# kelaendi/mused

Measured on AMD Instinct MI355X. Metric: stream rows/sec, d=1024 l=128 window=10k synthetic (SWFD + kNN similarity + eigenstep + labels), higher is better.
Workload: dtype f64; 1 GPU; synthetic d=1024 l=128 window=10000 k=50 (BASELINE config 2); stream=blob, W=10000, d=1024, l=128, k=50, modalities=1, swfd_levels=14, rccl_ranks=1, lanes_per_gpu=20, padded_window_slots=2

## Files before the change

mused_amd/csrc/gemm_f64.h:

```cpp
#pragma once
#include <cstdlib>
#include <mutex>
#include <type_traits>
#include "common.h"

namespace mused {

typedef double v4f64 __attribute__((ext_vector_type(4)));

constexpr int GEMM_BM = 128;
constexpr int GEMM_BN = 128;
constexpr int GEMM_BK = 16;
constexpr int GEMM_LD = 144;
constexpr int GEMM_THREADS = 256;
constexpr int GEMM_LDS_BYTES = 2  * 2  * GEMM_BK * GEMM_LD * 8;

struct GemmArgs {
  const void* A;
  const void* B;
  long lda, ldb;
  long strideA, strideB;
  int M, N, K;
  int kchunk;
  int splitk;
  int bsplit;
  int tiles_m, tiles_n;
  const int* rep;
  const int* list;
  const int* kact;
  int sym;
};

template <typename TIn, bool VEC>
__device__ __forceinline__ void stage_load_kc(const TIn* __restrict__ src, long ld, int r0, int nrows, int k0,
                                              int kend, TIn (&r)[8]) {
  const int m = threadIdx.x & 127;
  const int kh = threadIdx.x >> 7;
  const int row = r0 + m;
  const int k = k0 + kh * 8;
  if (row < nrows) {
    const TIn* p = src + (long)row * ld + k;
    if (VEC && k + 8 <= kend) {
      if (sizeof(TIn) == 4) {
        const float4 a = *reinterpret_cast<const float4*>(p);
        const float4 b = *reinterpret_cast<const float4*>(p + 4);
        r[0] = a.x; r[1] = a.y; r[2] = a.z; r[3] = a.w;
        r[4] = b.x; r[5] = b.y; r[6] = b.z; r[7] = b.w;
      } else {
        const double2* q = reinterpret_cast<const double2*>(p);
#pragma unroll
        for (int j = 0; j < 4; ++j) {
          const double2 v = q[j];
          r[2 * j] = v.x;
          r[2 * j + 1] = v.y;
        }
      }
    } else {
#pragma unroll
      for (int j = 0; j < 8; ++j) r[j] = (k + j < kend) ? p[j] : (TIn)0;
    }
  } else {
#pragma unroll
    for (int j = 0; j < 8; ++j) r[j] = (TIn)0;
// ... 52 lines not shown

template <typename TIn>
__device__ __forceinline__ void stage_load8(const TIn* __restrict__ p, TIn (&r)[8]) {
  if (sizeof(TIn) == 4) {
    const float4 a = *reinterpret_cast<const float4*>(p);
    const float4 b = *reinterpret_cast<const float4*>(p + 4);
    r[0] = a.x; r[1] = a.y; r[2] = a.z; r[3] = a.w;
    r[4] = b.x; r[5] = b.y; r[6] = b.z; r[7] = b.w;
  } else {
    const double2* q = reinterpret_cast<const double2*>(p);
#pragma unroll
    for (int j = 0; j < 4; ++j) {
      const double2 v = q[j];
      r[2 * j] = v.x;
      r[2 * j + 1] = v.y;
    }
  }
}
template <typename TIn>
__device__ __forceinline__ void stage_load_kc_full(const TIn* __restrict__ src, long ld, int r0, int k0, TIn (&r)[8]) {
  stage_load8(src + (long)(r0 + (threadIdx.x & 127)) * ld + k0 + (threadIdx.x >> 7) * 8, r);
}
template <typename TIn>
__device__ __forceinline__ void stage_load_mc_full(const TIn* __restrict__ src, long ld, int c0, int k0, TIn (&r)[8]) {
  stage_load8(src + (long)(k0 + (threadIdx.x >> 4)) * ld + c0 + (threadIdx.x & 15) * 8, r);
}

__device__ __forceinline__ int xcd_remap(int pid, int nwg) {
  const int q = nwg >> 3, r = nwg & 7, xcd = pid & 7;
  const int base = (xcd < r) ? xcd * (q + 1) : r * (q + 1) + (xcd - r) * q;
  return base + (pid >> 3);
}

template <typename TA, typename TB, bool A_KC, bool B_KC, bool VEC>
__device__ __forceinline__ void gemm_tile_mainloop(const GemmArgs& g, const TA* __restrict__ A, const TB* __restrict__ B,
                                                   int m0, int n0, int k_lo, int k_hi, double* smem,
                                                   v4f64 (&acc)[4][4]) {
  double* As = smem;
  double* Bs = smem + 2 * GEMM_BK * GEMM_LD;
  const int lane = threadIdx.x & 63;
  const int wave = threadIdx.x >> 6;
  const int wr = wave >> 1, wc = wave & 1;
  const int kq = lane >> 4, li = lane & 15;
#pragma unroll
  for (int i = 0; i < 4; ++i)
#pragma unroll
    for (int j = 0; j < 4; ++j) acc[i][j] = (v4f64){0.0, 0.0, 0.0, 0.0};

  TA ra[8];
  TB rb[8];
  const int nkt = (k_hi - k_lo + GEMM_BK - 1) / GEMM_BK;

  const bool full_mn = VEC && m0 + GEMM_BM <= g.M && n0 + GEMM_BN <= g.N;
  auto load_tile = [&](int kt) {
    const int k0 = k_lo + kt * GEMM_BK;
    if (full_mn && k0 + GEMM_BK <= k_hi) {
      if (A_KC) stage_load_kc_full<TA>(A, g.lda, m0, k0, ra); else stage_load_mc_full<TA>(A, g.lda, m0, k0, ra);
      if (B_KC) stage_load_kc_full<TB>(B, g.ldb, n0, k0, rb); else stage_load_mc_full<TB>(B, g.ldb, n0, k0, rb);
      return;
    }
    if (A_KC) stage_load_kc<TA, VEC>(A, g.lda, m0, g.M, k0, k_hi, ra);
    else      stage_load_mc<TA, VEC>(A, g.lda, m0, g.M, k0, k_hi, ra);
    if (B_KC) stage_load_kc<TB, VEC>(B, g.ldb, n0, g.N, k0, k_hi, rb);
    else      stage_load_mc<TB, VEC>(B, g.ldb, n0, g.N, k0, k_hi, rb);
  };
  auto store_tile = [&](int buf) {
    double* a = As + buf * GEMM_BK * GEMM_LD;
    double* b = Bs + buf * GEMM_BK * GEMM_LD;
    if (A_KC) stage_store_kc(a, ra); else stage_store_mc(a, ra);
    if (B_KC) stage_store_kc(b, rb); else stage_store_mc(b, rb);
  };

  if (nkt > 0) {
    load_tile(0);
    store_tile(0);
  }
  __syncthreads();

  int cur = 0;
  for (int kt = 0; kt < nkt; ++kt) {
    const bool more = (kt + 1 < nkt);
    if (more) load_tile(kt + 1);
    const double* a = As + cur * GEMM_BK * GEMM_LD + wr * 64 + li;
    const double* b = Bs + cur * GEMM_BK * GEMM_LD + wc * 64 + li;
#pragma unroll
    for (int kk = 0; kk < GEMM_BK / 4; ++kk) {
      double fa[4], fb[4];
#pragma unroll
      for (int i = 0; i < 4; ++i) fa[i] = a[(kk * 4 + kq) * GEMM_LD + i * 16];
#pragma unroll
      for (int j = 0; j < 4; ++j) fb[j] = b[(kk * 4 + kq) * GEMM_LD + j * 16];
#pragma unroll
      for (int i = 0; i < 4; ++i)
#pragma unroll
        for (int j = 0; j < 4; ++j)
          acc[i][j] = __builtin_amdgcn_mfma_f64_16x16x4f64(fa[i], fb[j], acc[i][j], 0, 0, 0);
    }
    if (more) store_tile(cur ^ 1);
    __syncthreads();
    cur ^= 1;
  }
}

constexpr int DIAG_I[4][9] = {{0, 0, 1, 0, 1, 2, 0, 1, 2}, {3, 0, 1, 2, 3, 4, 0, 1, 2}, {3, 4, 5, 0, 1, 2, 3, 4, 5}, {6, 0, 1, 2, 3, 4, 5, 6, 7}};
constexpr int DIAG_J[4][9] = {{0, 1, 1, 2, 2, 2, 3, 3, 3}, {3, 4, 4, 4, 4, 4, 5, 5, 5}, {5, 5, 5, 6, 6, 6, 6, 6, 6}, {6, 7, 7, 7, 7, 7, 7, 7, 7}};
constexpr int DIAG_NF[4] = {4, 6, 7, 8};
constexpr int DIAG_NGRP[4] = {3, 2, 2, 1};
constexpr int DIAG_GRP[4][3][3] = {{{1, 0, 1}, {2, 0, 2}, {3, 0, 3}}, {{4, 0, 4}, {5, 0, 3}, {0, 0, 0}}, {{5, 3, 2}, {6, 0, 6}, {0, 0, 0}}, {{7, 0, 7}, {0, 0, 0}, {0, 0, 0}}};
constexpr int DIAG_PATCH_LD = 130;

constexpr int diag_acc_index(int w, int i, int j) {
  for (int n = 0; n < 9; ++n)
    if (DIAG_I[w][n] == i && DIAG_J[w][n] == j) return n;
  return -1;
}

template <int W, int N = 0>
__device__ __forceinline__ void diag_mfma9(const double (&f)[8], v4f64 (&acc)[9]) {
  if constexpr (N < 9) {
    constexpr int i = DIAG_I[W][N], j = DIAG_J[W][N];
    acc[N] = __builtin_amdgcn_mfma_f64_16x16x4f64(f[i], f[j], acc[N], 0, 0, 0);
    diag_mfma9<W, N + 1>(f, acc);
  }
}
template <int W>
__device__ __forceinline__ void diag_kstep(const double* __restrict__ a, v4f64 (&acc)[9]) {
#pragma unroll
  for (int kk = 0; kk < GEMM_BK / 4; ++kk) {
    double f[8];
#pragma unroll
    for (int b = 0; b < 8; ++b) f[b] = (b < DIAG_NF[W]) ? a[kk * 4 * GEMM_LD + b * 16] : 0.0;
    diag_mfma9<W>(f, acc);
  }
}

template <typename TA, bool A_KC, bool VEC>
__device__ __forceinline__ void gemm_tile_mainloop_diag(const GemmArgs& g, const TA* __restrict__ A, int m0, int k_lo, int k_hi,
                                                        double* As, int wave, v4f64 (&acc)[9]) {
  const int lane = threadIdx.x & 63;
  const int kq = lane >> 4, li = lane & 15;
#pragma unroll
  for (int n = 0; n < 9; ++n) acc[n] = (v4f64){0.0, 0.0, 0.0, 0.0};

  TA ra[8];
  const int nkt = (k_hi - k_lo + GEMM_BK - 1) / GEMM_BK;
  const bool full_m = VEC && m0 + GEMM_BM <= g.M;
  auto load_tile = [&](int kt) {
    const int k0 = k_lo + kt * GEMM_BK;
    if (full_m && k0 + GEMM_BK <= k_hi) {
      if (A_KC) stage_load_kc_full<TA>(A, g.lda, m0, k0, ra); else stage_load_mc_full<TA>(A, g.lda, m0, k0, ra);
      return;
    }
    if (A_KC) stage_load_kc<TA, VEC>(A, g.lda, m0, g.M, k0, k_hi, ra);
    else      stage_load_mc<TA, VEC>(A, g.lda, m0, g.M, k0, k_hi, ra);
  };
  auto store_tile = [&](int buf) {
    double* a = As + buf * GEMM_BK * GEMM_LD;
    if (A_KC) stage_store_kc(a, ra); else stage_store_mc(a, ra);
  };

  if (nkt > 0) {
    load_tile(0);
    store_tile(0);
  }
  __syncthreads();

  int cur = 0;
  for (int kt = 0; kt < nkt; ++kt) {
    const bool more = (kt + 1 < nkt);
    if (more) load_tile(kt + 1);
    const double* a = As + cur * GEMM_BK * GEMM_LD + kq * GEMM_LD + li;
    switch (wave) {
      case 0: diag_kstep<0>(a, acc); break;
      case 1: diag_kstep<1>(a, acc); break;
      case 2: diag_kstep<2>(a, acc); break;
      default: diag_kstep<3>(a, acc); break;
    }
    if (more) store_tile(cur ^ 1);
    __syncthreads();
    cur ^= 1;
  }
}

template <int W, int GI, int II, typename Epi>
__device__ __forceinline__ void diag_mirror_fill(const GemmArgs& g, const Epi& epi, int m0, double* patch, const v4f64 (&acc)[9]) {
  constexpr int j = DIAG_GRP[W][GI][0], i0 = DIAG_GRP[W][GI][1], cnt = DIAG_GRP[W][GI][2];
  if constexpr (II < cnt) {
    constexpr int n = diag_acc_index(W, i0 + II, j);
    static_assert(n >= 0, "block not held by this wave");
    const int lane = threadIdx.x & 63;
    const int kq = lane >> 4, li = lane & 15;
    const int col = m0 + j * 16 + li;
#pragma unroll
    for (int r = 0; r < 4; ++r) {
      const int rl = II * 16 + kq + 4 * r;
      const int rg = m0 + i0 * 16 + rl;
      patch[li * DIAG_PATCH_LD + rl] = (rg < g.M && col < g.N) ? epi.value(col, rg, acc[n][r]) : 0.0;
    }
    diag_mirror_fill<W, GI, II + 1>(g, epi, m0, patch, acc);
  }
}

template <int W, int GI, typename Epi>
__device__ __forceinline__ void diag_mirror_groups(const GemmArgs& g, const Epi& epi, int z, int m0, double* patch,
                                                   const v4f64 (&acc)[9]) {
  if constexpr (GI < DIAG_NGRP[W]) {
    constexpr int j = DIAG_GRP[W][GI][0], i0 = DIAG_GRP[W][GI][1], cnt = DIAG_GRP[W][GI][2];
    constexpr int width = cnt * 16;
    const int lane = threadIdx.x & 63;
// ... 7 lines not shown
    }
    diag_mirror_groups<W, GI + 1>(g, epi, z, m0, patch, acc);
  }
}

template <int W, int N, typename Epi>
__device__ __forceinline__ void diag_store_blocks(const GemmArgs& g, const Epi& epi, int z, int m0, const v4f64 (&acc)[9]) {
  if constexpr (N < 9) {
    const int lane = threadIdx.x & 63;
    const int col = m0 + DIAG_J[W][N] * 16 + (lane & 15);
#pragma unroll
    for (int r = 0; r < 4; ++r) {
      const int row = m0 + DIAG_I[W][N] * 16 + (lane >> 4) + 4 * r;
      if (row < g.M && col < g.N) epi(z, row, col, acc[N][r]);
    }
    diag_store_blocks<W, N + 1>(g, epi, z, m0, acc);
  }
}

template <int W, typename Epi>
__device__ __forceinline__ void diag_epilogue(const GemmArgs& g, const Epi& epi, int z, int m0, double* smem,
                                              const v4f64 (&acc)[9]) {
  diag_store_blocks<W, 0>(g, epi, z, m0, acc);
  diag_mirror_groups<W, 0>(g, epi, z, m0, smem + W * (16 * DIAG_PATCH_LD), acc);
}

inline int gemm_sym_diag_enabled() {
  static const int on = [] {
    const char* s = getenv("MUSED_GEMM_SYM_DIAG");
    return (s && s[0] == '0') ? 0 : 1;
  }();
  return on;
}

template <typename TA, typename TB, bool A_KC, bool B_KC, bool VEC, typename Epi>
__global__ __launch_bounds__(GEMM_THREADS, 2) void gemm_f64_kernel(GemmArgs g, Epi epi) {
  extern __shared__ __attribute__((aligned(16))) double smem[];

  int z = blockIdx.z;
  int zb = g.bsplit ? z / g.bsplit : z;
  if (g.list) {
    if (zb >= g.list[0]) return;
    const int e = g.list[1 + zb];
    z += (e - zb) * (g.bsplit ? g.bsplit : 1);
    zb = e;
  } else if (g.rep && g.rep[zb] != zb) return;
  int tm, tn;
  if (g.sym) {
    const int t = g.tiles_n, nwg = t * (t + 1) / 2;
    const int e = xcd_remap(blockIdx.x, nwg);
    int r = (int)((2.0 * t + 1.0 - sqrt((2.0 * t + 1.0) * (2.0 * t + 1.0) - 8.0 * e)) * 0.5);
    r = r < 0 ? 0 : (r > t - 1 ? t - 1 : r);
    while (r > 0 && r * t - r * (r - 1) / 2 > e) --r;
    while (r + 1 < t && (r + 1) * t - (r + 1) * r / 2 <= e) ++r;
    tm = r;
    tn = r + (e - (r * t - r * (r - 1) / 2));
  } else {
    const int nwg = g.tiles_m * g.tiles_n;
    const int wg = xcd_remap(blockIdx.x, nwg);
    constexpr int GROUP_M = 8;
    const int per_group = GROUP_M * g.tiles_n;
    const int group_id = wg / per_group;
    const int first_m = group_id * GROUP_M;
    const int group_size = min(g.tiles_m - first_m, GROUP_M);
    tm = first_m + (wg % group_size);
    tn = (wg % per_group) / group_size;
  }
  const int m0 = tm * GEMM_BM, n0 = tn * GEMM_BN;
  const bool mirror = g.sym && tm != tn;

  int k_lo = 0, k_hi = g.K;
  const TA* A = reinterpret_cast<const TA*>(g.A);
  const TB* B = reinterpret_cast<const TB*>(g.B);
  if (g.splitk) {
    k_lo = z * g.kchunk;
    k_hi = min(g.K, k_lo + g.kchunk);
  } else {
    A += (long)zb * g.strideA;
    B += (long)zb * g.strideB;
    if (g.bsplit) {
      k_lo = (z - zb * g.bsplit) * g.kchunk;
      k_hi = min(g.K, k_lo + g.kchunk);
    } else if (g.kact) {
      k_hi = min(g.K, g.kact[zb]);
    }
  }

  if constexpr (std::is_same<TA, TB>::value && A_KC == B_KC) {
    if (g.sym == 2 && tm == tn) {
      const int w = __builtin_amdgcn_readfirstlane(threadIdx.x >> 6);
      v4f64 acc9[9];
      gemm_tile_mainloop_diag<TA, A_KC, VEC>(g, A, m0, k_lo, k_hi, smem, w, acc9);
      switch (w) {
        case 0: diag_epilogue<0>(g, epi, z, m0, smem, acc9); break;
        case 1: diag_epilogue<1>(g, epi, z, m0, smem, acc9); break;
        case 2: diag_epilogue<2>(g, epi, z, m0, smem, acc9); break;
        default: diag_epilogue<3>(g, epi, z, m0, smem, acc9); break;
      }
      return;
    }
  }

  const int lane = threadIdx.x & 63;
  const int wave = threadIdx.x >> 6;
  const int wr = wave >> 1, wc = wave & 1;
  const int kq = lane >> 4, li = lane & 15;

  v4f64 acc[4][4];
  gemm_tile_mainloop<TA, TB, A_KC, B_KC, VEC>(g, A, B, m0, n0, k_lo, k_hi, smem, acc);

#pragma unroll
  for (int i = 0; i < 4; ++i) {
#pragma unroll
    for (int j = 0; j < 4; ++j) {
      const int col = n0 + wc * 64 + j * 16 + li;
#pragma unroll
      for (int r = 0; r < 4; ++r) {
        const int row = m0 + wr * 64 + i * 16 + kq + 4 * r;
        if (row < g.M && col < g.N) epi(z, row, col, acc[i][j][r]);
      }
    }
  }
  if (mirror) {
    __syncthreads();
    double* patch = smem + wave * (32 * 65);
#pragma unroll
    for (int half = 0; half < 2; ++half) {
#pragma unroll
      for (int i = 0; i < 4; ++i)
#pragma unroll
        for (int jj = 0; jj < 2; ++jj) {
          const int j = half * 2 + jj;
          const int col = n0 + wc * 64 + j * 16 + li;
#pragma unroll
          for (int r = 0; r < 4; ++r) {
            const int rl = i * 16 + kq + 4 * r;
            const int rg = m0 + wr * 64 + rl;
            patch[(jj * 16 + li) * 65 + rl] = (rg < g.M && col < g.N) ? epi.value(col, rg, acc[i][j][r]) : 0.0;
          }
        }
      const int rowm = m0 + wr * 64 + lane;
#pragma unroll 8
      for (int c = 0; c < 32; ++c) {
        const int colm = n0 + wc * 64 + half * 32 + c;
        if (colm < g.N && rowm < g.M) epi.put(z, colm, rowm, patch[c * 65 + lane]);
      }
    }
  }
}

struct EpiStore {
  double* C;
  long ldc;
  long strideC;
  double alpha;
  __device__ __forceinline__ void operator()(int z, int row, int col, double v) const {
    C[(long)z * strideC + (long)row * ldc + col] = alpha * v;
  }
  __device__ __forceinline__ double value(int, int, double v) const { return alpha * v; }
  __device__ __forceinline__ void put(int z, int row, int col, double val) const {
    C[(long)z * strideC + (long)row * ldc + col] = val;
  }
};

template <typename TA, typename TB, bool A_KC, bool B_KC, bool VEC, typename Epi>
int gemm_f64_prepare_t() {
  static std::once_flag once;
  static hipError_t err = hipSuccess;
  std::call_once(once, [] {
    auto k = gemm_f64_kernel<TA, TB, A_KC, B_KC, VEC, Epi>;
    err = hipFuncSetAttribute(reinterpret_cast<const void*>(k), hipFuncAttributeMaxDynamicSharedMemorySize,
                              GEMM_LDS_BYTES);
  });
  MUSED_CHECK_HIP(err);
  return MUSED_OK;
}

template <typename TA, typename TB, bool A_KC, bool B_KC, typename Epi>
int gemm_f64_launch_t(GemmArgs g, int batch, Epi epi, bool vec, hipStream_t stream) {
  g.tiles_m = cdiv(g.M, GEMM_BM);
  g.tiles_n = cdiv(g.N, GEMM_BN);
  if (g.sym) g.sym = gemm_sym_diag_enabled() ? 2 : 1;
  if (g.M <= 0 || g.N <= 0 || batch <= 0) return MUSED_OK;
  dim3 grid(g.sym ? g.tiles_n * (g.tiles_n + 1) / 2 : g.tiles_m * g.tiles_n, 1, batch);
  int rc;
  if (vec) {
    if ((rc = gemm_f64_prepare_t<TA, TB, A_KC, B_KC, true, Epi>())) return rc;
    hipLaunchKernelGGL((gemm_f64_kernel<TA, TB, A_KC, B_KC, true, Epi>), grid, dim3(GEMM_THREADS), GEMM_LDS_BYTES,
                       stream, g, epi);
  } else {
    if ((rc = gemm_f64_prepare_t<TA, TB, A_KC, B_KC, false, Epi>())) return rc;
    hipLaunchKernelGGL((gemm_f64_kernel<TA, TB, A_KC, B_KC, false, Epi>), grid, dim3(GEMM_THREADS), GEMM_LDS_BYTES,
                       stream, g, epi);
  }
  MUSED_LAUNCH_CHECK();
  return MUSED_OK;
}

template <typename T>
static inline bool vec_ok(const void* p, long ld, long stride) {
  const long e = 16 / (long)sizeof(T);
  return ((uintptr_t)p % 16 == 0) && (ld % e == 0) && (stride % e == 0);
}

}
```

mused_amd/csrc/gemm_f64.hip:

```cpp
#include <stdarg.h>

#include "gemm_f64.h"
#include "internal.h"

namespace mused {

static thread_local char g_err[512] = "";

void set_error(const char* fmt, ...) {
  va_list ap;
  va_start(ap, fmt);
  vsnprintf(g_err, sizeof(g_err), fmt, ap);
  va_end(ap);
}

const char* last_error() { return g_err; }

int gemm_f64_prepare_all() {
  int rc = 0;
#define PREP(a, b, v) rc |= gemm_f64_prepare_t<double, double, a, b, v, EpiStore>()
  PREP(true, true, true); PREP(true, true, false); PREP(true, false, true); PREP(true, false, false);
  PREP(false, true, true); PREP(false, true, false); PREP(false, false, true); PREP(false, false, false);
#undef PREP
  return rc ? MUSED_ERR_HIP : MUSED_OK;
}

int gemm_f64(bool a_kc, bool b_kc, const double* A, long lda, long strideA, const double* B, long ldb,
             long strideB, double* C, long ldc, long strideC, int M, int N, int K, int batch, double alpha,
             hipStream_t stream, const int* rep, const int* list, const int* kact) {
  GemmArgs g;
  memset(&g, 0, sizeof(g));
  g.A = A; g.B = B; g.lda = lda; g.ldb = ldb; g.strideA = strideA; g.strideB = strideB;
  g.M = M; g.N = N; g.K = K; g.splitk = 0; g.kchunk = 0;
  g.rep = rep; g.list = list; g.kact = kact;
  g.sym = (A == B && a_kc == b_kc && lda == ldb && strideA == strideB && M == N) ? 1 : 0;
  EpiStore epi{C, ldc, strideC, alpha};
  const bool vec = vec_ok<double>(A, lda, strideA) && vec_ok<double>(B, ldb, strideB);
  if (a_kc && b_kc) return gemm_f64_launch_t<double, double, true, true>(g, batch, epi, vec, stream);
  if (a_kc && !b_kc) return gemm_f64_launch_t<double, double, true, false>(g, batch, epi, vec, stream);
  if (!a_kc && b_kc) return gemm_f64_launch_t<double, double, false, true>(g, batch, epi, vec, stream);
  return gemm_f64_launch_t<double, double, false, false>(g, batch, epi, vec, stream);
}

int gemm_f64_splitk(bool a_kc, bool b_kc, const double* A, long lda, const double* B, long ldb, double* partial,
                    int M, int N, int K, int kchunk, int nsplit, hipStream_t stream) {
  MUSED_REQUIRE(kchunk > 0 && kchunk % GEMM_BK == 0 && nsplit >= 1 && (long)kchunk * nsplit >= K,
                "gemm_f64_splitk: bad kchunk %d x %d for K=%d", kchunk, nsplit, K);
  GemmArgs g;
  memset(&g, 0, sizeof(g));
  g.A = A; g.B = B; g.lda = lda; g.ldb = ldb;
  g.M = M; g.N = N; g.K = K; g.splitk = 1; g.kchunk = kchunk;
  EpiStore epi{partial, (long)N, (long)M * N, 1.0};
  const bool vec = vec_ok<double>(A, lda, 0) && vec_ok<double>(B, ldb, 0);
  if (a_kc && b_kc) return gemm_f64_launch_t<double, double, true, true>(g, nsplit, epi, vec, stream);
  if (a_kc && !b_kc) return gemm_f64_launch_t<double, double, true, false>(g, nsplit, epi, vec, stream);
  if (!a_kc && b_kc) return gemm_f64_launch_t<double, double, false, true>(g, nsplit, epi, vec, stream);
  return gemm_f64_launch_t<double, double, false, false>(g, nsplit, epi, vec, stream);
}

__global__ void splitk_reduce_kernel(const double* __restrict__ partial, int nsplit, long count,
                                     double* __restrict__ out) {
  const long i = (long)blockIdx.x * blockDim.x + threadIdx.x;
  if (i >= count) return;
  double s = 0.0;
  for (int z = 0; z < nsplit; ++z) s += partial[(long)z * count + i];
  out[i] = s;
}

int gemm_f64_batched_splitk(bool a_kc, bool b_kc, const double* A, long lda, long strideA, const double* B, long ldb, long strideB,
                            double* partial, int M, int N, int K, int batch, int kchunk, int nsplit, hipStream_t stream,
                            const int* rep, const int* list) {
  MUSED_REQUIRE(kchunk > 0 && kchunk % GEMM_BK == 0 && nsplit >= 1 && (long)kchunk * nsplit >= K,
                "gemm_f64_batched_splitk: bad kchunk %d x %d for K=%d", kchunk, nsplit, K);
  GemmArgs g;
  memset(&g, 0, sizeof(g));
  g.A = A; g.B = B; g.lda = lda; g.ldb = ldb; g.strideA = strideA; g.strideB = strideB;
  g.M = M; g.N = N; g.K = K; g.splitk = 0; g.kchunk = kchunk; g.bsplit = nsplit;
  g.rep = rep; g.list = list;
  g.sym = (A == B && a_kc == b_kc && lda == ldb && strideA == strideB && M == N) ? 1 : 0;
  EpiStore epi{partial, (long)N, (long)M * N, 1.0};
  const bool vec = vec_ok<double>(A, lda, strideA) && vec_ok<double>(B, ldb, strideB);
  if (a_kc && b_kc) return gemm_f64_launch_t<double, double, true, true>(g, batch * nsplit, epi, vec, stream);
  if (a_kc && !b_kc) return gemm_f64_launch_t<double, double, true, false>(g, batch * nsplit, epi, vec, stream);
  if (!a_kc && b_kc) return gemm_f64_launch_t<double, double, false, true>(g, batch * nsplit, epi, vec, stream);
  return gemm_f64_launch_t<double, double, false, false>(g, batch * nsplit, epi, vec, stream);
}

__global__ void batched_splitk_reduce_kernel(const double* __restrict__ partial, int nsplit, long count, double* __restrict__ out,
                                             const int* __restrict__ rep, const int* __restrict__ list) {
  int z = blockIdx.y;
  if (list) {
    if (z >= list[0]) return;
    z = list[1 + z];
  } else if (rep && rep[z] != z) return;
  const long i = (long)blockIdx.x * blockDim.x + threadIdx.x;
  if (i >= count) return;
  const double* p = partial + (long)z * nsplit * count + i;
  double s = 0.0;
  for (int sp = 0; sp < nsplit; ++sp) s += p[(long)sp * count];
  out[(long)z * count + i] = s;
}

int gemm_batched_splitk_reduce(const double* partial, int nsplit, long count, double* out, int batch, const int* rep,
                               hipStream_t stream, const int* list) {
  hipLaunchKernelGGL(batched_splitk_reduce_kernel, dim3(cdiv(count, 256), batch), dim3(256), 0, stream, partial, nsplit, count, out,
                     rep, list);
  MUSED_LAUNCH_CHECK();
  return MUSED_OK;
}

int gemm_splitk_reduce(const double* partial, int nsplit, long count, double* out, hipStream_t stream) {
// ... 14 lines not shown
int mused_memcpy_d2d(void* dst, const void* src, long bytes, void* stream) {
  MUSED_REQUIRE(dst && src && bytes >= 0, "mused_memcpy_d2d: bad arguments");
  MUSED_CHECK_HIP(hipMemcpyAsync(dst, src, (size_t)bytes, hipMemcpyDeviceToDevice, (hipStream_t)stream));
  return MUSED_OK;
}

int mused_gemm_f64(int a_kc, int b_kc, const double* A, long lda, const double* B, long ldb, double* C, long ldc,
                   int M, int N, int K, double alpha, void* stream) {
  return mused::gemm_f64(a_kc != 0, b_kc != 0, A, lda, 0, B, ldb, 0, C, ldc, 0, M, N, K, 1, alpha,
                         (hipStream_t)stream);
}

int mused_gemm_f64_batched(int a_kc, int b_kc, const double* A, long lda, long strideA, const double* B, long ldb,
                           long strideB, double* C, long ldc, long strideC, int M, int N, int K, int batch,
                           double alpha, void* stream) {
  return mused::gemm_f64(a_kc != 0, b_kc != 0, A, lda, strideA, B, ldb, strideB, C, ldc, strideC, M, N, K, batch,
                         alpha, (hipStream_t)stream);
}

int mused_gemm_f64_batched_rep(int a_kc, int b_kc, const double* A, long lda, long strideA, const double* B, long ldb,
                               long strideB, double* C, long ldc, long strideC, int M, int N, int K, int batch,
                               double alpha, const int* rep, void* stream) {
  return mused::gemm_f64(a_kc != 0, b_kc != 0, A, lda, strideA, B, ldb, strideB, C, ldc, strideC, M, N, K, batch,
                         alpha, (hipStream_t)stream, rep);
}

int mused_debug_gemm_f64_batched_active(int a_kc, int b_kc, const double* A, long lda, long strideA, const double* B, long ldb,
                                        long strideB, double* C, long ldc, long strideC, int M, int N, int K, int batch,
                                        double alpha, const int* list, const int* kact, void* stream) {
  return mused::gemm_f64(a_kc != 0, b_kc != 0, A, lda, strideA, B, ldb, strideB, C, ldc, strideC, M, N, K, batch,
                         alpha, (hipStream_t)stream, nullptr, list, kact);
}

int mused_gemm_f64_splitk(int a_kc, int b_kc, const double* A, long lda, const double* B, long ldb, double* partial,
                          double* C, int M, int N, int K, int kchunk, int nsplit, void* stream) {
  MUSED_REQUIRE(A && B && partial && C && M >= 0 && N >= 0 && K >= 0, "mused_gemm_f64_splitk: bad arguments");
  int rc = mused::gemm_f64_splitk(a_kc != 0, b_kc != 0, A, lda, B, ldb, partial, M, N, K, kchunk, nsplit,
                                  (hipStream_t)stream);
  if (rc != MUSED_OK || M == 0 || N == 0) return rc;
  return mused::gemm_splitk_reduce(partial, nsplit, (long)M * N, C, (hipStream_t)stream);
}

int mused_gemm_f64_batched_splitk(int a_kc, int b_kc, const double* A, long lda, long strideA, const double* B, long ldb,
                                  long strideB, double* partial, double* C, int M, int N, int K, int batch, int kchunk,
                                  int nsplit, const int* rep, void* stream) {
  MUSED_REQUIRE(A && B && partial && C && M >= 0 && N >= 0 && K >= 0 && batch >= 1,
                "mused_gemm_f64_batched_splitk: bad arguments");
  int rc = mused::gemm_f64_batched_splitk(a_kc != 0, b_kc != 0, A, lda, strideA, B, ldb, strideB, partial, M, N, K, batch,
                                          kchunk, nsplit, (hipStream_t)stream, rep);
  if (rc != MUSED_OK || M == 0 || N == 0) return rc;
  return mused::gemm_batched_splitk_reduce(partial, nsplit, (long)M * N, C, batch, rep, (hipStream_t)stream);
}

}
```

mused_amd/csrc/internal.h:

```cpp
#pragma once
#include "common.h"

#include <mutex>

namespace mused {

int select_from_records(const double* rec, int n, int kind, int k, int* out_idx, unsigned long long* out_mask,
                        int mask_words, hipStream_t stream);
int select_from_tag_sets(const int* rowptr, const int* tags, const int* postptr, const int* postrow, int n, int k,
                         int* out_idx, unsigned long long* out_mask, int mask_words, hipStream_t stream);
int select_max_fused_rows(bool tag_sets);
int select_window_records(const double* rec, const int* vrank, int s, int e, int kind, int k, unsigned long long* out_mask,
                          int mask_words, hipStream_t stream);
int select_window_tag_sets(const int* rowptr, const int* tags, const int* postptr, const int* postrow, const int* vrank, int s,
                           int e, int k, unsigned long long* out_mask, int mask_words, hipStream_t stream);

std::recursive_mutex& capture_mutex();
using CaptureLock = std::lock_guard<std::recursive_mutex>;


int gemm_f64(bool a_kc, bool b_kc, const double* A, long lda, long strideA, const double* B, long ldb,
             long strideB, double* C, long ldc, long strideC, int M, int N, int K, int batch, double alpha,
             hipStream_t stream, const int* rep = nullptr, const int* list = nullptr, const int* kact = nullptr);

int gemm_f64_batched_splitk(bool a_kc, bool b_kc, const double* A, long lda, long strideA, const double* B, long ldb, long strideB,
                            double* partial, int M, int N, int K, int batch, int kchunk, int nsplit, hipStream_t stream,
                            const int* rep = nullptr, const int* list = nullptr);
int gemm_batched_splitk_reduce(const double* partial, int nsplit, long count, double* out, int batch, const int* rep,
                               hipStream_t stream, const int* list = nullptr);
int gemm_f64_prepare_all();

int gemm_f64_splitk(bool a_kc, bool b_kc, const double* A, long lda, const double* B, long ldb, double* partial,
                    int M, int N, int K, int kchunk, int nsplit, hipStream_t stream);
int gemm_splitk_reduce(const double* partial, int nsplit, long count, double* out, hipStream_t stream);

int lu_permute_l(double* Y, int n, int r, long ld, int* pivstep, double* prow, long ws_f64_len, hipStream_t st);
int qr_economic(double* Y, int n, int r, long ldy, double* Q, long ldq, double* tau, double* wpart, hipStream_t st,
                const int* run_if = nullptr);
int spmm_binary(const int* rowptr, const int* colidx, int n, const double* Q, long ldq, int r, double* Y, long ldy,
                hipStream_t stream, const double* col_sign = nullptr);

int spmm_valued(const int* rowptr, const int* colidx, const double* vals, int n, const double* Q, long ldq, int r, double* Y,
                long ldy, hipStream_t stream, const double* col_sign = nullptr);

constexpr int ADJ_VAL_MAX_M = 8;
struct AdjValSrc {
  const void* p[ADJ_VAL_MAX_M];
  double w[ADJ_VAL_MAX_M];
  long ld;
  int M, dtype;
};
int adj_val_src_masks(const unsigned long long* const* masks, const double* weights, int M, AdjValSrc* out, const char* who);
int adj_val_src_dense(const void* dense, int dtype, int n, long ld, AdjValSrc* out, const char* who);
int adj_val_src_store(const AdjValSrc& src, AdjValSrc* dst, hipStream_t st);
int adj_csr_values_dev(const AdjValSrc* src_dev, bool dense, int n, int words, const int* rowptr, const int* colidx,
                       int transposed, double* vals, int* flag, hipStream_t st);

int adj_csr_from_mask(const unsigned long long* mask, int n, int words, int* deg, int* rowptr, int* colidx,
                      int* stats, long cap, int* overflow, hipStream_t st);
int zero_ints(int* p, long n, hipStream_t st);
// ... 48 lines not shown
```

mused_amd/csrc/swfd.hip:

```cpp
#include <vector>

#include "internal.h"

namespace mused {

struct Swfd {
  int N, d, ell, L, S, cap, n2, n4, n3;
  int lanes;
  double R;
  long i;
  int pend;
  long restart_mark;
  int skip_dead;
  bool twin;
  int sweeps;
  double* buf;
  bool tail_dirty;
  bool settle;
  int* used;
  double* queue;
  long long* qt;
  int* meta;
  int* rep;
  int* list;
  int* offs;
  int oround;
  int* kact;
  long long* ostat;
  long long* dropped;
  double* theta;
  double *T, *Wc;
  int gram_split;
  double* gpart;
  int* plan;
  int* keep_src;
  long long* now_dev;
  int* status;
  int* status_host;
  EigPlan* eig;
  double *stack, *Wq, *Bout, *sig_out, *qinfo;
  int* qsel;
  EigPlan* eigq;
  EigPlan* eigq3;
  int pre_chunk;
  double *pre_in, *pre_out, *pre_gram;
  EigPlan* eigp;
};

static inline int sk_index(const Swfd* h, int lane, int level, int kind) { return lane * 2 * h->L + kind * h->L + level; }

struct BitWord { unsigned long long w; };
template <typename T>
__device__ __forceinline__ double row_elem(const T* row, int c) { return (double)row[c]; }
template <>
__device__ __forceinline__ double row_elem<BitWord>(const BitWord* row, int c) {
  return (double)((row[c >> 6].w >> (c & 63)) & 1ull);
}

template <typename T>
__device__ __forceinline__ double2 row_pair(const T* row, int c);
// ... 285 lines not shown
  const int rho = blockIdx.x, s = blockIdx.y;
  const int sr = rep ? rep[s] : s;
  const int nk = meta[s * 4 + 0];
  if (sr < 0) {
    if (rho < nxt && nk + rho < n2)
      row_copy<Src>(buf + ((long)s * n2 + nk + rho) * d, X + (long)(s / per_lane) * lane_stride + (long)rho * ldx, d);
    return;
  }
  const double* Ts = T + (long)sr * ell * d;
  if (rho < ell && plan[(s * ell + rho) * 2] == 2) {
    const int slot = plan[(s * ell + rho) * 2 + 1];
    row_copy<double>(queue + ((long)s * cap + slot) * d, Ts + (long)rho * d, d);
  }
  double* dst = buf + ((long)s * n2 + rho) * d;
  if (rho < nk) {
    row_copy<double>(dst, Ts + (long)keep_src[s * ell + rho] * d, d);
  } else if (rho < nk + nxt) {
    row_copy<Src>(dst, X + (long)(s / per_lane) * lane_stride + (long)(rho - nk) * ldx, d);
  } else if (rho < (fill_all ? n2 : used[s])) {
    row_zero(dst, d);
  }
}

template <typename Src>
static int swfd_rotate_all(Swfd* h, hipStream_t st, const Src* next, long ldx, long lane_stride, int nxt) {
  const int S = h->S, n2 = h->n2, d = h->d, ell = h->ell;
  int rc;
  if (h->rep)
    hipLaunchKernelGGL(swfd_rep_kernel, dim3(1), dim3(1024), sizeof(int) * (size_t)S, st, h->meta, h->L, 2 * h->lanes, h->rep,
                       h->twin ? 1 : 0, h->dropped, (long long)(((h->i - 1) / h->N) * h->N), h->skip_dead, h->now_dev,
                       (long long)h->i, h->pend, ell, n2, h->list, h->offs, h->kact, h->ostat, h->oround);
  else
    hipLaunchKernelGGL(swfd_set_now_kernel, dim3(1), dim3(1), 0, st, h->now_dev, (long long)h->i);
  if (h->gram_split > 1) {
    const int kchunk = ((d + h->gram_split - 1) / h->gram_split + 15) / 16 * 16;
    if ((rc = gemm_f64_batched_splitk(true, true, h->buf, d, (long)n2 * d, h->buf, d, (long)n2 * d, h->gpart, n2, n2, d, S, kchunk,
                                      h->gram_split, st, h->rep, h->list)))
      return rc;
    if ((rc = gemm_batched_splitk_reduce(h->gpart, h->gram_split, (long)n2 * n2, eig_plan_input(h->eig), S, h->rep, st, h->list)))
      return rc;
  } else if ((rc = gemm_f64(true, true, h->buf, d, (long)n2 * d, h->buf, d, (long)n2 * d, eig_plan_input(h->eig), n2,
                            (long)n2 * n2, n2, n2, d, S, 1.0, st, h->rep, h->list)))
    return rc;
  if ((rc = eig_plan_run_inplace(h->eig, nullptr, nullptr, st, true))) return rc;
  const EigColumns e = eig_plan_columns(h->eig);
  hipLaunchKernelGGL(swfd_decide_kernel, dim3(S), dim3(1024), 0, st, e.lam, e.cols, e.ld, n2, ell, h->cap, h->N, h->now_dev,
                     h->theta, h->meta, h->qt, h->dropped, h->plan, h->keep_src, h->Wc, h->rep, h->settle ? h->used : nullptr,
                     h->pend);
  if ((rc = gemm_f64(true, false, h->Wc, n2, (long)ell * n2, h->buf, d, (long)n2 * d, h->T, d, (long)ell * d, ell, d,
                     n2, S, 1.0, st, h->rep, h->list, h->kact)))
    return rc;
  if (h->settle) {
    hipLaunchKernelGGL(swfd_settle_kernel<Src>, dim3(n2, S), dim3(256), 0, st, h->T, h->plan, h->keep_src, h->meta, h->used,
                       h->tail_dirty ? 1 : 0, h->buf, h->queue, n2, ell, h->cap, d, h->rep, next, ldx, lane_stride, 2 * h->L,
                       nxt);
    h->tail_dirty = false;
  } else {
    hipLaunchKernelGGL(swfd_scatter_kernel, dim3(n2, S), dim3(256), 0, st, h->T, h->plan, h->keep_src, h->meta, h->buf,
                       h->queue, n2, ell, h->cap, d, h->rep);
  }
  MUSED_LAUNCH_CHECK();
  h->pend = 0;
  return MUSED_OK;
}

static int swfd_restart(Swfd* h, hipStream_t st) {
  const long be = (long)h->n2 * h->d, qe = (long)h->cap * h->d;
  const long m = be > qe ? be : qe;
  hipLaunchKernelGGL(swfd_restart_kernel, dim3(cdiv(m, 256), h->L * h->lanes), dim3(256), 0, st, h->buf, h->queue, h->qt,
                     h->meta, h->dropped, h->L, be, qe, h->cap);
  MUSED_LAUNCH_CHECK();
  return MUSED_OK;
}

constexpr int SWFD_PRE_MAX = 96;
// ... 309 lines not shown
  double r1 = R > 1.0 ? R : 1.0;
  int lg = 0;
  while ((double)(1ull << lg) < r1 && lg < 62) ++lg;
  h->L = lg + 1;
  h->lanes = lanes;
  h->S = 2 * h->L * lanes;
  MUSED_REQUIRE(h->S <= 8192, "mused_swfd_create: %d sketches (lanes x 2 levels), at most 8192", h->S);
  h->cap = 2 * ell;
  h->n2 = 2 * ell;
  h->n4 = 4 * ell;
  h->n3 = (3 * ell + 1) & ~1;
  h->sweeps = sweeps > 0 ? sweeps : 24;
  h->restart_mark = -1;
  h->twin = true;
  const size_t S = h->S, n2 = h->n2, n4 = h->n4, cap = h->cap, dd = d, l = ell;
#define ALLOC(p, bytes) MUSED_CHECK_HIP(hipMalloc((void**)&(p), (bytes)))
#define ZALLOC(p, bytes) do { ALLOC(p, bytes); MUSED_CHECK_HIP(hipMemset((p), 0, (bytes))); } while (0)
  ZALLOC(h->buf, 8 * S * n2 * dd);
  ZALLOC(h->queue, 8 * S * cap * dd);
  ZALLOC(h->qt, 8 * S * cap);
  ZALLOC(h->meta, 4 * S * 4);
  {
    const char* dd = getenv("MUSED_SWFD_DEDUPE");
    if (!(dd && dd[0] == '0')) ALLOC(h->rep, 4 * S);
    auto off = [](const char* name) { const char* v = getenv(name); return v && v[0] == '0'; };
    if (h->rep && !off("MUSED_SWFD_LIST")) {
      ZALLOC(h->list, 4 * (S + 1));
      ZALLOC(h->ostat, 8 * 18);
      if (!off("MUSED_SWFD_ORDERS")) ZALLOC(h->offs, 4 * S);
      const char* orr = getenv("MUSED_SWFD_ORDERS");
      const int rv = orr ? atoi(orr) : 0;
      h->oround = (rv == 1 || rv == 16 || rv == 32) ? rv : SWFD_OFFS_ROUND;
      if (!off("MUSED_SWFD_KACT")) ZALLOC(h->kact, 4 * S);
    }
    const char* sd = getenv("MUSED_SWFD_SKIP_DEAD");
    h->skip_dead = (sd && sd[0] == '0') ? 0 : 1;
    h->settle = !off("MUSED_SWFD_SETTLE");
    if (h->settle) ZALLOC(h->used, 4 * S);
  }
  ZALLOC(h->dropped, 8 * S);
  ZALLOC(h->status, 4);
  MUSED_CHECK_HIP(hipHostMalloc((void**)&h->status_host, sizeof(int), hipHostMallocDefault));
  ALLOC(h->theta, 8 * S);
  ALLOC(h->T, 8 * S * l * dd); ALLOC(h->Wc, 8 * S * l * n2);
  ALLOC(h->plan, 4 * S * l * 2); ALLOC(h->keep_src, 4 * S * l); ALLOC(h->now_dev, 8);
  {
    const char* gs = getenv("MUSED_SWFD_GRAM_SPLIT");
    h->gram_split = gs ? atoi(gs) : (d >= 8192 ? 8 : 1);
    if (h->gram_split < 1 || h->gram_split > 16) h->gram_split = 1;
    if (h->gram_split > 1) ALLOC(h->gpart, 8 * S * (size_t)h->gram_split * n2 * n2);
  }
  const size_t Bn = lanes;
  ALLOC(h->stack, 8 * Bn * n4 * dd);
  ALLOC(h->Wq, 8 * Bn * l * n4); ALLOC(h->Bout, 8 * Bn * l * dd); ALLOC(h->sig_out, 8 * Bn * l);
  ALLOC(h->qinfo, 8 * 2 * Bn); ALLOC(h->qsel, 4 * Bn * (4 + cap));
#undef ZALLOC
#undef ALLOC
  std::vector<double> th(S);
  for (int lane = 0; lane < lanes; ++lane)
    for (int kind = 0; kind < 2; ++kind)
      for (int j = 0; j < h->L; ++j) th[sk_index(h, lane, j, kind)] = ldexp((double)h->N / ell, j);
  MUSED_CHECK_HIP(hipMemcpy(h->theta, th.data(), 8 * S, hipMemcpyHostToDevice));
  int rc;
  if ((rc = gemm_f64_prepare_all())) return rc;
  if ((rc = eig_plan_create(h->n2, h->S, h->sweeps, true, &h->eig, h->rep, EIG_PLAN_TOP_HALF, h->status, 0, h->list, h->offs)))
    return rc;
// ... 228 lines not shown
```

Before: 652,000 rows/s.

## Skip inactive rows/cols in symmetric SWFD Gram GEMM using per-batch active count

```diff
diff --git a/mused_amd/csrc/gemm_f64.h b/mused_amd/csrc/gemm_f64.h
--- a/mused_amd/csrc/gemm_f64.h
+++ b/mused_amd/csrc/gemm_f64.h
@@ -29,6 +29,7 @@
   const int* list;
   const int* kact;
   int sym;
+  const int* nact;
 };
 
 template <typename TIn, bool VEC>
@@ -147,10 +148,25 @@
   return base + (pid >> 3);
 }
 
-template <typename TA, typename TB, bool A_KC, bool B_KC, bool VEC>
+template <int NJ>
+__device__ __forceinline__ void tile_kstep(const double* __restrict__ a, const double* __restrict__ b, v4f64 (&acc)[4][4]) {
+#pragma unroll
+  for (int kk = 0; kk < GEMM_BK / 4; ++kk) {
+    double fa[4], fb[4];
+#pragma unroll
+    for (int i = 0; i < 4; ++i) fa[i] = a[kk * 4 * GEMM_LD + i * 16];
+#pragma unroll
+    for (int j = 0; j < 4; ++j) fb[j] = (j < NJ) ? b[kk * 4 * GEMM_LD + j * 16] : 0.0;
+#pragma unroll
+    for (int i = 0; i < 4; ++i)
+#pragma unroll
+      for (int j = 0; j < NJ; ++j) acc[i][j] = __builtin_amdgcn_mfma_f64_16x16x4f64(fa[i], fb[j], acc[i][j], 0, 0, 0);
+  }
+}
+template <typename TA, typename TB, bool A_KC, bool B_KC, bool VEC, bool BND = false>
 __device__ __forceinline__ void gemm_tile_mainloop(const GemmArgs& g, const TA* __restrict__ A, const TB* __restrict__ B,
                                                    int m0, int n0, int k_lo, int k_hi, double* smem,
-                                                   v4f64 (&acc)[4][4]) {
+                                                   v4f64 (&acc)[4][4], int nb = 0) {
   double* As = smem;
   double* Bs = smem + 2 * GEMM_BK * GEMM_LD;
   const int lane = threadIdx.x & 63;
@@ -166,6 +182,13 @@
   TB rb[8];
   const int nkt = (k_hi - k_lo + GEMM_BK - 1) / GEMM_BK;
 
+  int nj = 4, rows_a = g.M, rows_b = g.N;
+  if (BND) {
+    const int aj = (nb - n0 - (__builtin_amdgcn_readfirstlane(wave) & 1) * 64 + 15) >> 4;
+    nj = aj < 0 ? 0 : (aj > 4 ? 4 : aj);
+    rows_a = min(g.M, nb);
+    rows_b = min(g.N, nb);
+  }
   const bool full_mn = VEC && m0 + GEMM_BM <= g.M && n0 + GEMM_BN <= g.N;
   auto load_tile = [&](int kt) {
     const int k0 = k_lo + kt * GEMM_BK;
@@ -174,10 +197,10 @@
       if (B_KC) stage_load_kc_full<TB>(B, g.ldb, n0, k0, rb); else stage_load_mc_full<TB>(B, g.ldb, n0, k0, rb);
       return;
     }
-    if (A_KC) stage_load_kc<TA, VEC>(A, g.lda, m0, g.M, k0, k_hi, ra);
-    else      stage_load_mc<TA, VEC>(A, g.lda, m0, g.M, k0, k_hi, ra);
-    if (B_KC) stage_load_kc<TB, VEC>(B, g.ldb, n0, g.N, k0, k_hi, rb);
-    else      stage_load_mc<TB, VEC>(B, g.ldb, n0, g.N, k0, k_hi, rb);
+    if (A_KC) stage_load_kc<TA, VEC>(A, g.lda, m0, rows_a, k0, k_hi, ra);
+    else      stage_load_mc<TA, VEC>(A, g.lda, m0, rows_a, k0, k_hi, ra);
+    if (B_KC) stage_load_kc<TB, VEC>(B, g.ldb, n0, rows_b, k0, k_hi, rb);
+    else      stage_load_mc<TB, VEC>(B, g.ldb, n0, rows_b, k0, k_hi, rb);
   };
   auto store_tile = [&](int buf) {
     double* a = As + buf * GEMM_BK * GEMM_LD;
@@ -192,28 +215,29 @@
   }
   __syncthreads();
 
-  int cur = 0;
-  for (int kt = 0; kt < nkt; ++kt) {
-    const bool more = (kt + 1 < nkt);
-    if (more) load_tile(kt + 1);
-    const double* a = As + cur * GEMM_BK * GEMM_LD + wr * 64 + li;
-    const double* b = Bs + cur * GEMM_BK * GEMM_LD + wc * 64 + li;
-#pragma unroll
-    for (int kk = 0; kk < GEMM_BK / 4; ++kk) {
-      double fa[4], fb[4];
-#pragma unroll
-      for (int i = 0; i < 4; ++i) fa[i] = a[(kk * 4 + kq) * GEMM_LD + i * 16];
-#pragma unroll
-      for (int j = 0; j < 4; ++j) fb[j] = b[(kk * 4 + kq) * GEMM_LD + j * 16];
-#pragma unroll
-      for (int i = 0; i < 4; ++i)
-#pragma unroll
-        for (int j = 0; j < 4; ++j)
-          acc[i][j] = __builtin_amdgcn_mfma_f64_16x16x4f64(fa[i], fb[j], acc[i][j], 0, 0, 0);
-    }
-    if (more) store_tile(cur ^ 1);
-    __syncthreads();
-    cur ^= 1;
+  auto kloop = [&](auto njc) {
+    constexpr int NJ = decltype(njc)::value;
+    int cur = 0;
+    for (int kt = 0; kt < nkt; ++kt) {
+      const bool more = (kt + 1 < nkt);
+      if (more) load_tile(kt + 1);
+      const double* a = As + cur * GEMM_BK * GEMM_LD + wr * 64 + li;
+      const double* b = Bs + cur * GEMM_BK * GEMM_LD + wc * 64 + li;
+      tile_kstep<NJ>(a + kq * GEMM_LD, b + kq * GEMM_LD, acc);
+      if (more) store_tile(cur ^ 1);
+      __syncthreads();
+      cur ^= 1;
+    }
+  };
+  if (BND && nj < 4) {
+    switch (nj) {
+      case 3: kloop(std::integral_constant<int, 3>{}); break;
+      case 2: kloop(std::integral_constant<int, 2>{}); break;
+      case 1: kloop(std::integral_constant<int, 1>{}); break;
+      default: kloop(std::integral_constant<int, 0>{}); break;
+    }
+  } else {
+    kloop(std::integral_constant<int, 4>{});
   }
 }
 
@@ -230,28 +254,51 @@
   return -1;
 }
 
-template <int W, int N = 0>
+template <int W, int CNT, int N = 0>
 __device__ __forceinline__ void diag_mfma9(const double (&f)[8], v4f64 (&acc)[9]) {
-  if constexpr (N < 9) {
+  if constexpr (N < CNT) {
     constexpr int i = DIAG_I[W][N], j = DIAG_J[W][N];
     acc[N] = __builtin_amdgcn_mfma_f64_16x16x4f64(f[i], f[j], acc[N], 0, 0, 0);
-    diag_mfma9<W, N + 1>(f, acc);
-  }
-}
-template <int W>
+    diag_mfma9<W, CNT, N + 1>(f, acc);
+  }
+}
+template <int W, int CNT>
 __device__ __forceinline__ void diag_kstep(const double* __restrict__ a, v4f64 (&acc)[9]) {
 #pragma unroll
   for (int kk = 0; kk < GEMM_BK / 4; ++kk) {
     double f[8];
 #pragma unroll
-    for (int b = 0; b < 8; ++b) f[b] = (b < DIAG_NF[W]) ? a[kk * 4 * GEMM_LD + b * 16] : 0.0;
-    diag_mfma9<W>(f, acc);
-  }
-}
-
-template <typename TA, bool A_KC, bool VEC>
+    for (int b = 0; b < 8; ++b) f[b] = (b < DIAG_NF[W] && b <= DIAG_J[W][CNT - 1]) ? a[kk * 4 * GEMM_LD + b * 16] : 0.0;
+    diag_mfma9<W, CNT>(f, acc);
+  }
+}
+template <int W, int C>
+__device__ __forceinline__ void diag_stage_cnt(const double* __restrict__ a, v4f64 (&acc)[9], int cnt) {
+  if constexpr (C >= 1) {
+    if constexpr (C == 9 || DIAG_J[W][C == 9 ? 8 : C] != DIAG_J[W][C - 1]) {
+      if (cnt == C) {
+        diag_kstep<W, C>(a, acc);
+        return;
+      }
+    }
+    diag_stage_cnt<W, C - 1>(a, acc, cnt);
+  }
+}
+template <int W, bool BND>
+__device__ __forceinline__ void diag_stage(const double* __restrict__ a, v4f64 (&acc)[9], int m0, int nb) {
+  if (!BND) {
+    diag_kstep<W, 9>(a, acc);
+    return;
+  }
+  int cnt = 0;
+#pragma unroll
+  for (int n = 0; n < 9; ++n) cnt += (m0 + DIAG_J[W][n] * 16 < nb) ? 1 : 0;
+  diag_stage_cnt<W, 9>(a, acc, cnt);
+}
+
+template <typename TA, bool A_KC, bool VEC, bool BND>
 __device__ __forceinline__ void gemm_tile_mainloop_diag(const GemmArgs& g, const TA* __restrict__ A, int m0, int k_lo, int k_hi,
-                                                        double* As, int wave, v4f64 (&acc)[9]) {
+                                                        double* As, int wave, v4f64 (&acc)[9], int nb) {
   const int lane = threadIdx.x & 63;
   const int kq = lane >> 4, li = lane & 15;
 #pragma unroll
@@ -260,14 +307,15 @@
   TA ra[8];
   const int nkt = (k_hi - k_lo + GEMM_BK - 1) / GEMM_BK;
   const bool full_m = VEC && m0 + GEMM_BM <= g.M;
+  const int rows = BND ? min(g.M, nb) : g.M;
   auto load_tile = [&](int kt) {
     const int k0 = k_lo + kt * GEMM_BK;
     if (full_m && k0 + GEMM_BK <= k_hi) {
       if (A_KC) stage_load_kc_full<TA>(A, g.lda, m0, k0, ra); else stage_load_mc_full<TA>(A, g.lda, m0, k0, ra);
       return;
     }
-    if (A_KC) stage_load_kc<TA, VEC>(A, g.lda, m0, g.M, k0, k_hi, ra);
-    else      stage_load_mc<TA, VEC>(A, g.lda, m0, g.M, k0, k_hi, ra);
+    if (A_KC) stage_load_kc<TA, VEC>(A, g.lda, m0, rows, k0, k_hi, ra);
+    else      stage_load_mc<TA, VEC>(A, g.lda, m0, rows, k0, k_hi, ra);
   };
   auto store_tile = [&](int buf) {
     double* a = As + buf * GEMM_BK * GEMM_LD;
@@ -286,10 +334,10 @@
     if (more) load_tile(kt + 1);
     const double* a = As + cur * GEMM_BK * GEMM_LD + kq * GEMM_LD + li;
     switch (wave) {
-      case 0: diag_kstep<0>(a, acc); break;
-      case 1: diag_kstep<1>(a, acc); break;
-      case 2: diag_kstep<2>(a, acc); break;
-      default: diag_kstep<3>(a, acc); break;
+      case 0: diag_stage<0, BND>(a, acc, m0, nb); break;
+      case 1: diag_stage<1, BND>(a, acc, m0, nb); break;
+      case 2: diag_stage<2, BND>(a, acc, m0, nb); break;
+      default: diag_stage<3, BND>(a, acc, m0, nb); break;
     }
     if (more) store_tile(cur ^ 1);
     __syncthreads();
@@ -363,8 +411,7 @@
   }();
   return on;
 }
-
-template <typename TA, typename TB, bool A_KC, bool B_KC, bool VEC, typename Epi>
+template <typename TA, typename TB, bool A_KC, bool B_KC, bool VEC, typename Epi, bool BOUNDS = false>
 __global__ __launch_bounds__(GEMM_THREADS, 2) void gemm_f64_kernel(GemmArgs g, Epi epi) {
   extern __shared__ __attribute__((aligned(16))) double smem[];
 
@@ -416,12 +463,17 @@
       k_hi = min(g.K, g.kact[zb]);
     }
   }
+  int nb = g.M > g.N ? g.M : g.N;
+  if (BOUNDS) {
+    nb = min(nb, g.nact[zb]);
+    if (m0 >= nb || n0 >= nb) k_hi = k_lo;
+  }
 
   if constexpr (std::is_same<TA, TB>::value && A_KC == B_KC) {
     if (g.sym == 2 && tm == tn) {
       const int w = __builtin_amdgcn_readfirstlane(threadIdx.x >> 6);
       v4f64 acc9[9];
-      gemm_tile_mainloop_diag<TA, A_KC, VEC>(g, A, m0, k_lo, k_hi, smem, w, acc9);
+      gemm_tile_mainloop_diag<TA, A_KC, VEC, BOUNDS>(g, A, m0, k_lo, k_hi, smem, w, acc9, nb);
       switch (w) {
         case 0: diag_epilogue<0>(g, epi, z, m0, smem, acc9); break;
         case 1: diag_epilogue<1>(g, epi, z, m0, smem, acc9); break;
@@ -438,7 +490,10 @@
   const int kq = lane >> 4, li = lane & 15;
 
   v4f64 acc[4][4];
-  gemm_tile_mainloop<TA, TB, A_KC, B_KC, VEC>(g, A, B, m0, n0, k_lo, k_hi, smem, acc);
+  if (BOUNDS && n0 + GEMM_BN > nb && k_hi > k_lo)
+    gemm_tile_mainloop<TA, TB, A_KC, B_KC, VEC, true>(g, A, B, m0, n0, k_lo, k_hi, smem, acc, nb);
+  else
+    gemm_tile_mainloop<TA, TB, A_KC, B_KC, VEC>(g, A, B, m0, n0, k_lo, k_hi, smem, acc);
 
 #pragma unroll
   for (int i = 0; i < 4; ++i) {
@@ -494,12 +549,12 @@
   }
 };
 
-template <typename TA, typename TB, bool A_KC, bool B_KC, bool VEC, typename Epi>
+template <typename TA, typename TB, bool A_KC, bool B_KC, bool VEC, typename Epi, bool BOUNDS = false>
 int gemm_f64_prepare_t() {
   static std::once_flag once;
   static hipError_t err = hipSuccess;
   std::call_once(once, [] {
-    auto k = gemm_f64_kernel<TA, TB, A_KC, B_KC, VEC, Epi>;
+    auto k = gemm_f64_kernel<TA, TB, A_KC, B_KC, VEC, Epi, BOUNDS>;
     err = hipFuncSetAttribute(reinterpret_cast<const void*>(k), hipFuncAttributeMaxDynamicSharedMemorySize,
                               GEMM_LDS_BYTES);
   });
@@ -512,9 +567,26 @@
   g.tiles_m = cdiv(g.M, GEMM_BM);
   g.tiles_n = cdiv(g.N, GEMM_BN);
   if (g.sym) g.sym = gemm_sym_diag_enabled() ? 2 : 1;
+  if (!g.sym || g.splitk) g.nact = nullptr;
   if (g.M <= 0 || g.N <= 0 || batch <= 0) return MUSED_OK;
   dim3 grid(g.sym ? g.tiles_n * (g.tiles_n + 1) / 2 : g.tiles_m * g.tiles_n, 1, batch);
   int rc;
+  if constexpr (std::is_same<TA, TB>::value && A_KC == B_KC && std::is_same<Epi, EpiStore>::value) {
+    if (g.nact) {
+      if (vec) {
+        if ((rc = gemm_f64_prepare_t<TA, TB, A_KC, B_KC, true, Epi, true>())) return rc;
+        hipLaunchKernelGGL((gemm_f64_kernel<TA, TB, A_KC, B_KC, true, Epi, true>), grid, dim3(GEMM_THREADS), GEMM_LDS_BYTES,
+                           stream, g, epi);
+      } else {
+        if ((rc = gemm_f64_prepare_t<TA, TB, A_KC, B_KC, false, Epi, true>())) return rc;
+        hipLaunchKernelGGL((gemm_f64_kernel<TA, TB, A_KC, B_KC, false, Epi, true>), grid, dim3(GEMM_THREADS), GEMM_LDS_BYTES,
+                           stream, g, epi);
+      }
+      MUSED_LAUNCH_CHECK();
+      return MUSED_OK;
+    }
+  }
+  g.nact = nullptr;
   if (vec) {
     if ((rc = gemm_f64_prepare_t<TA, TB, A_KC, B_KC, true, Epi>())) return rc;
     hipLaunchKernelGGL((gemm_f64_kernel<TA, TB, A_KC, B_KC, true, Epi>), grid, dim3(GEMM_THREADS), GEMM_LDS_BYTES,
diff --git a/mused_amd/csrc/gemm_f64.hip b/mused_amd/csrc/gemm_f64.hip
--- a/mused_amd/csrc/gemm_f64.hip
+++ b/mused_amd/csrc/gemm_f64.hip
@@ -22,17 +22,21 @@
   PREP(true, true, true); PREP(true, true, false); PREP(true, false, true); PREP(true, false, false);
   PREP(false, true, true); PREP(false, true, false); PREP(false, false, true); PREP(false, false, false);
 #undef PREP
+  rc |= gemm_f64_prepare_t<double, double, true, true, true, EpiStore, true>();
+  rc |= gemm_f64_prepare_t<double, double, true, true, false, EpiStore, true>();
+  rc |= gemm_f64_prepare_t<double, double, false, false, true, EpiStore, true>();
+  rc |= gemm_f64_prepare_t<double, double, false, false, false, EpiStore, true>();
   return rc ? MUSED_ERR_HIP : MUSED_OK;
 }
 
 int gemm_f64(bool a_kc, bool b_kc, const double* A, long lda, long strideA, const double* B, long ldb,
              long strideB, double* C, long ldc, long strideC, int M, int N, int K, int batch, double alpha,
-             hipStream_t stream, const int* rep, const int* list, const int* kact) {
+             hipStream_t stream, const int* rep, const int* list, const int* kact, const int* nact) {
   GemmArgs g;
   memset(&g, 0, sizeof(g));
   g.A = A; g.B = B; g.lda = lda; g.ldb = ldb; g.strideA = strideA; g.strideB = strideB;
   g.M = M; g.N = N; g.K = K; g.splitk = 0; g.kchunk = 0;
-  g.rep = rep; g.list = list; g.kact = kact;
+  g.rep = rep; g.list = list; g.kact = kact; g.nact = nact;
   g.sym = (A == B && a_kc == b_kc && lda == ldb && strideA == strideB && M == N) ? 1 : 0;
   EpiStore epi{C, ldc, strideC, alpha};
   const bool vec = vec_ok<double>(A, lda, strideA) && vec_ok<double>(B, ldb, strideB);
@@ -69,14 +73,14 @@
 
 int gemm_f64_batched_splitk(bool a_kc, bool b_kc, const double* A, long lda, long strideA, const double* B, long ldb, long strideB,
                             double* partial, int M, int N, int K, int batch, int kchunk, int nsplit, hipStream_t stream,
-                            const int* rep, const int* list) {
+                            const int* rep, const int* list, const int* nact) {
   MUSED_REQUIRE(kchunk > 0 && kchunk % GEMM_BK == 0 && nsplit >= 1 && (long)kchunk * nsplit >= K,
                 "gemm_f64_batched_splitk: bad kchunk %d x %d for K=%d", kchunk, nsplit, K);
   GemmArgs g;
   memset(&g, 0, sizeof(g));
   g.A = A; g.B = B; g.lda = lda; g.ldb = ldb; g.strideA = strideA; g.strideB = strideB;
   g.M = M; g.N = N; g.K = K; g.splitk = 0; g.kchunk = kchunk; g.bsplit = nsplit;
-  g.rep = rep; g.list = list;
+  g.rep = rep; g.list = list; g.nact = nact;
   g.sym = (A == B && a_kc == b_kc && lda == ldb && strideA == strideB && M == N) ? 1 : 0;
   EpiStore epi{partial, (long)N, (long)M * N, 1.0};
   const bool vec = vec_ok<double>(A, lda, strideA) && vec_ok<double>(B, ldb, strideB);
@@ -157,6 +161,25 @@
                          alpha, (hipStream_t)stream, nullptr, list, kact);
 }
 
+int mused_debug_gemm_f64_batched_bounds(int a_kc, int b_kc, const double* A, long lda, long strideA, const double* B, long ldb,
+                                        long strideB, double* C, long ldc, long strideC, int M, int N, int K, int batch,
+                                        double alpha, const int* list, const int* kact, const int* nact, void* stream) {
+  return mused::gemm_f64(a_kc != 0, b_kc != 0, A, lda, strideA, B, ldb, strideB, C, ldc, strideC, M, N, K, batch,
+                         alpha, (hipStream_t)stream, nullptr, list, kact, nact);
+}
+
+int mused_debug_gemm_f64_batched_splitk_bounds(int a_kc, int b_kc, const double* A, long lda, long strideA, const double* B,
+                                               long ldb, long strideB, double* partial, double* C, int M, int N, int K,
+                                               int batch, int kchunk, int nsplit, const int* list, const int* nact,
+                                               void* stream) {
+  MUSED_REQUIRE(A && B && partial && C && M > 0 && N > 0 && K >= 0 && batch >= 1,
+                "mused_debug_gemm_f64_batched_splitk_bounds: bad arguments");
+  int rc = mused::gemm_f64_batched_splitk(a_kc != 0, b_kc != 0, A, lda, strideA, B, ldb, strideB, partial, M, N, K, batch,
+                                          kchunk, nsplit, (hipStream_t)stream, nullptr, list, nact);
+  if (rc != MUSED_OK) return rc;
+  return mused::gemm_batched_splitk_reduce(partial, nsplit, (long)M * N, C, batch, nullptr, (hipStream_t)stream, list);
+}
+
 int mused_gemm_f64_splitk(int a_kc, int b_kc, const double* A, long lda, const double* B, long ldb, double* partial,
                           double* C, int M, int N, int K, int kchunk, int nsplit, void* stream) {
   MUSED_REQUIRE(A && B && partial && C && M >= 0 && N >= 0 && K >= 0, "mused_gemm_f64_splitk: bad arguments");
diff --git a/mused_amd/csrc/internal.h b/mused_amd/csrc/internal.h
--- a/mused_amd/csrc/internal.h
+++ b/mused_amd/csrc/internal.h
@@ -21,11 +21,12 @@
 
 int gemm_f64(bool a_kc, bool b_kc, const double* A, long lda, long strideA, const double* B, long ldb,
              long strideB, double* C, long ldc, long strideC, int M, int N, int K, int batch, double alpha,
-             hipStream_t stream, const int* rep = nullptr, const int* list = nullptr, const int* kact = nullptr);
+             hipStream_t stream, const int* rep = nullptr, const int* list = nullptr, const int* kact = nullptr,
+             const int* nact = nullptr);
 
 int gemm_f64_batched_splitk(bool a_kc, bool b_kc, const double* A, long lda, long strideA, const double* B, long ldb, long strideB,
                             double* partial, int M, int N, int K, int batch, int kchunk, int nsplit, hipStream_t stream,
-                            const int* rep = nullptr, const int* list = nullptr);
+                            const int* rep = nullptr, const int* list = nullptr, const int* nact = nullptr);
 int gemm_batched_splitk_reduce(const double* partial, int nsplit, long count, double* out, int batch, const int* rep,
                                hipStream_t stream, const int* list = nullptr);
 int gemm_f64_prepare_all();
diff --git a/mused_amd/csrc/swfd.hip b/mused_amd/csrc/swfd.hip
--- a/mused_amd/csrc/swfd.hip
+++ b/mused_amd/csrc/swfd.hip
@@ -26,6 +26,7 @@
   int* offs;
   int oround;
   int* kact;
+  bool nact;
   long long* ostat;
   long long* dropped;
   double* theta;
@@ -377,6 +378,7 @@
                        (long long)h->i, h->pend, ell, n2, h->list, h->offs, h->kact, h->ostat, h->oround);
   else
     hipLaunchKernelGGL(swfd_set_now_kernel, dim3(1), dim3(1), 0, st, h->now_dev, (long long)h->i);
+  const int* nact = (h->nact && !h->tail_dirty) ? h->kact : nullptr;
   if (h->gram_split > 1) {
     const int kchunk = ((d + h->gram_split - 1) / h->gram_split + 15) / 16 * 16;
     if ((rc = gemm_f64_batched_splitk(true, true, h->buf, d, (long)n2 * d, h->buf, d, (long)n2 * d, h->gpart, n2, n2, d, S, kchunk,
@@ -385,7 +387,7 @@
     if ((rc = gemm_batched_splitk_reduce(h->gpart, h->gram_split, (long)n2 * n2, eig_plan_input(h->eig), S, h->rep, st, h->list)))
       return rc;
   } else if ((rc = gemm_f64(true, true, h->buf, d, (long)n2 * d, h->buf, d, (long)n2 * d, eig_plan_input(h->eig), n2,
-                            (long)n2 * n2, n2, n2, d, S, 1.0, st, h->rep, h->list)))
+                            (long)n2 * n2, n2, n2, d, S, 1.0, st, h->rep, h->list, nullptr, nact)))
     return rc;
   if ((rc = eig_plan_run_inplace(h->eig, nullptr, nullptr, st, true))) return rc;
   const EigColumns e = eig_plan_columns(h->eig);
@@ -761,6 +763,7 @@
       const int rv = orr ? atoi(orr) : 0;
       h->oround = (rv == 1 || rv == 16 || rv == 32) ? rv : SWFD_OFFS_ROUND;
       if (!off("MUSED_SWFD_KACT")) ZALLOC(h->kact, 4 * S);
+      h->nact = h->kact && !off("MUSED_SWFD_NACT");
     }
     const char* sd = getenv("MUSED_SWFD_SKIP_DEAD");
     h->skip_dead = (sd && sd[0] == '0') ? 0 : 1;
```

Result: no change. 654,000 rows/s, median of 6 (+0.3%).
